# Parcels-code/Parcels

Hardware: AMD Instinct MI355X
Metric: RK4 particle-steps/sec (higher is better)
Workload: dtype f64

## Files before the change

parcels_amd/csrc/pk_api.hip:

```cpp
#include "pk_api_ctx.h"

#include <rocprim/rocprim.hpp>

using namespace pkapi;

namespace pkapi {
std::string g_init_error;
}

namespace pk {

PK_DEV unsigned long long order_double(double v) {
    unsigned long long b = (unsigned long long)__double_as_longlong(v);
    return (b & 0x8000000000000000ull) ? ~b : (b | 0x8000000000000000ull);
}

__global__ void __launch_bounds__(64) clock_probe_kernel(unsigned long long* out, unsigned long long ticks) {
    if (threadIdx.x != 0) return;
    const unsigned long long r0 = __builtin_amdgcn_s_memrealtime();
    const unsigned long long c0 = __builtin_readcyclecounter();
    unsigned long long r = r0;
    while (r - r0 < ticks) {
        __builtin_amdgcn_s_sleep(8);
        r = __builtin_amdgcn_s_memrealtime();
// ... 1701 lines not shown
    if (ok) {
        PK_HIP(ctx, hipStreamSynchronize(ctx->compute));
        if (tab.size() > t.cap) {
            if (t.d) PK_HIP(ctx, hipFree(t.d));
            PK_HIP(ctx, hipMalloc((void**)&t.d, tab.size() * sizeof(double)));
            t.cap = tab.size();
        }
        PK_HIP(ctx, hipMemcpy(t.d, tab.data(), tab.size() * sizeof(double), hipMemcpyHostToDevice));
    }
    t.ok = ok;
    return 0;
}

static int32_t fill_fast(pk_ctx* ctx, const pk_exec_params* prm, KArgs& a, int prog) {
    FastA& F = a.fast;
    memset(&F, 0, sizeof(F));
    if (ctx->no_fast || prm->interp_uv != 0 || prm->rk45_mode) return 0;
    const bool want_w = prog == PROG_RK4_3D;
    const HostField& U = ctx->fields[prm->fU];
    const HostField& V = ctx->fields[prm->fV];
    const HostField* W = (want_w && prm->fW >= 0) ? &ctx->fields[prm->fW] : nullptr;
    if (want_w && !W) return 0;
    const HostGrid& g = ctx->grids[U.d.grid];
    if (g.d.kind != 0 || g.d.lon_f32 || g.d.lat_f32 || g.d.depth_f32) return 0;
    if (V.d.grid != U.d.grid || (W && W->d.grid != U.d.grid)) return 0;
    auto same = [](const DField& x, const DField& y) { return x.ncomp == 1 && y.ncomp == 1 && same_layout(x, y); };
    if (!same(U.d, V.d) || (W && !same(U.d, W->d))) return 0;
    if (V.time != U.time || (W && W->time != U.time)) return 0;
    const DField& f = U.d;
    const size_t esz = f.dtype == PK_F64 ? 8 : 4;
    if (!g.d.has_x || f.st_x != 1 || f.nx < 2 || f.nx != g.d.nx) return 0;
    const bool fy = f.ny >= 2 && f.st_y > 0, fz = f.nz >= 2 && f.st_z > 0;
    if (fy && !(g.d.has_y && f.ny == g.d.ny)) return 0;
    if (fz && !(g.d.has_z && f.nz == g.d.nz)) return 0;
    if (f.has_time_interval && (f.nt < 2 || U.time.front() != 0.0)) return 0;
    const uint64_t lvl_b = (uint64_t)f.st_t * esz;
    const uint64_t last_b = ((uint64_t)f.nz * (uint64_t)f.st_z + (uint64_t)f.ny * (uint64_t)f.st_y + (uint64_t)f.nx) * esz;
    if (lvl_b >= (1ull << 32) || last_b >= (1ull << 32)) return 0;
    const CoordTable& T = ctx->tab_a;
    if (int32_t rc = coord_table(ctx, ctx->tab_a, U.d.grid, prm->fU, U.time.data(), f.has_time_interval ? f.nt : 0,
                                 {{g.d.depth, g.d.has_z ? g.d.nz : 0}, {g.d.lat, g.d.has_y ? g.d.ny : 0}, {g.d.lon, g.d.nx}}, 60 * 1024))
        return rc;
    if (!T.ok) return 0;
    const double inv_deg2m = 1.0 / g.d.deg2m;
    if (!(g.d.deg2m > 1e-100 && g.d.deg2m < 1e100) || !std::isfinite(inv_deg2m)) return 0;
    F.grid = U.d.grid;
    F.has_ti = f.has_time_interval;
    F.has_z = g.d.has_z; F.has_y = g.d.has_y; F.has_x = g.d.has_x;
    F.spherical = g.d.spherical;
    F.nt = f.nt;
    F.nslots = f.nslots;
    F.gnz = g.d.nz; F.gny = g.d.ny; F.gnx = g.d.nx;
    ravel_strides(g.d, F.ex, F.ey, F.ez);
    F.st_z = (uint32_t)f.st_z;
    F.st_y = (uint32_t)f.st_y;
    F.dyb = fy ? (uint32_t)(f.st_y * esz) : 0u;
    F.dzb = fz ? (uint32_t)(f.st_z * esz) : 0u;
    F.lds_time = T.off[0]; F.lds_depth = T.off[1]; F.lds_lat = T.off[2]; F.lds_lon = T.off[3];
    F.lds_n = T.off[4];
    F.lvl_b = (int64_t)lvl_b;
    F.U = (const char*)U.d.data; F.V = (const char*)V.d.data; F.W = W ? (const char*)W->d.data : nullptr;
    F.tab = T.d;
    F.tlen = f.tlen; F.t0 = f.tfirst; F.t1 = f.tlast;
    F.z0 = g.d.zfirst; F.z1 = g.d.zlast; F.y0 = g.d.yfirst; F.y1 = g.d.ylast; F.x0 = g.d.xfirst; F.x1 = g.d.xlast;
    F.deg2m = g.d.deg2m;
    F.inv_deg2m = inv_deg2m;
    F.ok = 1;
    return 0;
}

static void ensure_velocity_pairs(pk_ctx* ctx, const pk_exec_params* prm, FastC& F) {
    F.vp = nullptr;
    F.vp_slot_b = 0;
    F.vp_hi = 0;
    if (ctx->no_velocity_pairs) return;
    const HostField& U = ctx->fields[prm->fU];
    const HostField& V = ctx->fields[prm->fV];
    const DField& f = U.d;
    if (!f.has_time_interval || f.nt < 2 || f.st_t <= 0) return;
    const size_t esz = f.dtype == PK_F64 ? 8 : 4;
    const int ns = f.nslots;
    const size_t slot_b = (size_t)f.st_t * 8 * esz;
    const size_t need = slot_b * (size_t)ns;
    if (ctx->vp_fU != prm->fU || ctx->vp_fV != prm->fV || ctx->vp_bytes != need || (int)ctx->vp_level.size() != ns) {
        if (ctx->d_vp) {
            (void)hipStreamSynchronize(ctx->compute);
            (void)hipFree(ctx->d_vp);
            ctx->d_vp = nullptr;
        }
        ctx->vp_fU = prm->fU;
        ctx->vp_fV = prm->fV;
        ctx->vp_bytes = need;
        ctx->vp_level.assign(ns, -1);
        ctx->vp_gen.assign((size_t)ns * 4, 0);
        size_t free_b = 0, total_b = 0;
        if (hipMemGetInfo(&free_b, &total_b) != hipSuccess || free_b < need + std::max(need, total_b / 4)) {
            (void)hipGetLastError();
            ctx->d_vp = nullptr;
        } else if (hipMalloc((void**)&ctx->d_vp, need) != hipSuccess) {
            (void)hipGetLastError();
            ctx->d_vp = nullptr;
        }
    }
    if (!ctx->d_vp) return;
    const int64_t cb = F.cb;
    int lo = -1, hi = -1, count = 0;
// ... 664 lines not shown
```

parcels_amd/csrc/pk_device.h:

```cpp
#pragma once
#include <hip/hip_runtime.h>
#include <stdint.h>

#include "../../include/parcels_hip.h"

namespace pk {

struct DGrid {
    int32_t kind, spherical;
    int32_t has_x, has_y, has_z;
    int32_t nx, ny, nz;
    int32_t xdim, ydim, zdim;
    int32_t off_x, off_y, off_z;
    int32_t lon_f32, lat_f32, depth_f32;
    int32_t h_bitwidth;
    double deg2m;
    const double* lon;
    const double* lat;
    const double* depth;
    const double* node_tab;
    const double* cell_tab;
    const uint32_t* h_keys;
    const int64_t* h_starts;
    const int64_t* h_counts;
// ... 25 lines not shown
    int32_t ngrids, spatial_f32;
    double* t;
    void *z, *y, *x, *dz, *dy, *dx;
    double* dt;
    double* next_dt;
    int32_t* state;
    int32_t* ei;
    int64_t* particle_id;
    void* extra[PK_MAX_EXTRA];
    int32_t extra_f32[PK_MAX_EXTRA];
    int32_t* iter;
};

struct DPOut {
    double* t;
    void *z, *y, *x, *dz, *dy, *dx;
    double* dt;
    double* next_dt;
    int32_t* state;
    int32_t* ei;
    int32_t* iter;
};

struct DCounters {
    unsigned long long steps, attempts, paused;
    unsigned int err_iter, pad;
    unsigned long long twe_key;
    unsigned int twe_overflow, pad2;
    unsigned int pad3[20];
    unsigned int cursor[8 * 32];
};
constexpr int PK_CURSOR_STRIDE = 32;
static_assert(offsetof(DCounters, cursor) == 128, "the cursors start on a line of their own");

struct FastA {
    int32_t ok, grid;
    int32_t has_ti, has_z, has_y, has_x, spherical;
    int32_t nt, nslots;
    int32_t gnz, gny, gnx;
    uint32_t ex, ey, ez;
    uint32_t st_z, st_y;
    uint32_t dyb, dzb;
    int32_t lds_time, lds_depth, lds_lat, lds_lon, lds_n;
    int32_t lds_blk;
    int64_t lvl_b;
    const char *U, *V, *W;
    const double* tab;
    double tlen, t0, t1, z0, z1, y0, y1, x0, x1;
    double deg2m, inv_deg2m;
    int32_t ns;
    int32_t miss_lanes;
    int32_t sfid[4];
    const char* S[4];
};

struct FastC {
    int32_t ok, grid;
    int32_t has_ti, has_z, walk_ok, near_edges;
    int32_t nt, nslots;
    int32_t gnz, gny, gnx;
    uint32_t ex, ey, ez;
    int32_t lds_time, lds_depth, lds_n;
    int32_t lds_rec, lds_fv;
    int32_t st_z, st_y;
    int32_t cb;
    int64_t lvl_b;
    int64_t dU0, dU1, dV0, dV1;
    union { int64_t dW0; int64_t vp_slot_b; };
    union { int64_t dW1; int64_t vp_hi; };
    const char *U, *V;
    union { const char* W; const char* vp; };
    const char* kh[2];
    int32_t kh_st[2], kh_sz[2], kh_sy[2];
    int32_t kh_nt[2], kh_nz[2], kh_ny[2], kh_nx[2], kh_has_ti[2], kh_nslots[2];
    const double* ct2;
    const double* tab;
    double tlen, t0, t1, z0, z1, deg2m;
};

struct SigmaA {
    const double* tab;
    int32_t n;
    int32_t fh, fzeta;
    int32_t cs_f32;
    double hc;
};

#define PK_CONST_AS __attribute__((address_space(4)))
struct KArgs {
    const PK_CONST_AS DGrid* grids;
    const PK_CONST_AS DField* fields;
    DParticles p;
    pk_exec_params prm;
    double win_lo, win_hi;
    DCounters* counters;
    const unsigned long long* twe_listed;
    unsigned long long* twe_found;
    unsigned int* twe_hit;
    int32_t lds_time, lds_depth, lds_lat, lds_lon, lds_total;
    int32_t lds_cc_nodes, lds_cc_keys, lds_cc_fvals;
    int32_t main_grid, main_field;
    DPOut po;
    union {
        FastA fast;
        FastC fastc;
        SigmaA sigma;
    };
};

#define PK_DEV __device__ __forceinline__
PK_DEV const DGrid& kgrid(const KArgs& a, int g) { return *(const DGrid*)(a.grids + g); }
PK_DEV const DField& kfield(const KArgs& a, int f) { return *(const DField*)(a.fields + f); }
PK_DEV unsigned long long twe_sample_key(unsigned it, int klo) { return ((unsigned long long)it << 32) | (unsigned long long)(unsigned)klo; }
PK_DEV bool twe_listed(const KArgs& a, unsigned it, int klo) {
    const int n = a.prm.twe_n;
    if (__builtin_expect(n == 0, 1)) return false;
    const unsigned long long key = twe_sample_key(it, klo);
    const unsigned long long* lst = a.twe_listed;
    int lo = 0, hi = n;
    while (lo < hi) {
        const int mid = (lo + hi) >> 1;
        if (lst[mid] < key) lo = mid + 1; else hi = mid;
    }
    return it != 0 && lo < n && lst[lo] == key;
}
PK_DEV void twe_note(const KArgs& a, unsigned it, int klo) {
    if (it != 0) atomicMin(&a.counters->twe_key, twe_sample_key(it, klo));
}
constexpr int TWE_FOUND_SLOTS = 4096;
PK_DEV void twe_note_all(const KArgs& a, unsigned it, int klo) {
    if (it == 0) return;
    const unsigned long long key = twe_sample_key(it, klo);
    atomicMin(&a.counters->twe_key, key);
    unsigned h = (unsigned)((key * 0x9E3779B97F4A7C15ull) >> 52);
    for (int probe = 0; probe < TWE_FOUND_SLOTS; probe++) {
        unsigned long long* slot = a.twe_found + ((h + probe) & (TWE_FOUND_SLOTS - 1));
        unsigned long long cur = *(volatile unsigned long long*)slot;
        if (cur == key) return;
        if (cur == 0ull) {
            cur = atomicCAS(slot, 0ull, key);
            if (cur == 0ull || cur == key) return;
        }
    }
    atomicAdd(&a.counters->twe_overflow, 1u);
}
PK_DEV int twe_listed_index(const KArgs& a, unsigned it, int klo) {
    const int n = a.prm.twe_n;
    if (__builtin_expect(n == 0, 1)) return -1;
    const unsigned long long key = twe_sample_key(it, klo);
    const unsigned long long* lst = a.twe_listed;
    int lo = 0, hi = n;
    while (lo < hi) {
        const int mid = (lo + hi) >> 1;
        if (lst[mid] < key) lo = mid + 1; else hi = mid;
    }
    return (it != 0 && lo < n && lst[lo] == key) ? lo : -1;
}
PK_DEV void twe_justify(const KArgs& a, int idx, double t, double tlen) {
    if (!(0 <= t) || !(t <= tlen)) a.twe_hit[idx] = 1u;
}

// ... 1360 lines not shown
```

parcels_amd/csrc/pk_fast_agrid.h:

```cpp
#pragma once
#include "pk_device.h"

namespace pk {

typedef double pk_tab2 __attribute__((ext_vector_type(2)));

struct FastTabs {
    const pk_tab2* time;
    const pk_tab2* depth;
    const pk_tab2* lat;
    const pk_tab2* lon;
    pk_tab2* blk;
    uint32_t fl;
    double tlen;
    int32_t gny, gnx;
    double deg2m, inv_deg2m;
};
PK_DEV void copy_scalars(FastTabs& T, const FastA& F) {
    T.tlen = F.tlen;
    T.gny = F.gny;
    T.gnx = F.gnx;
}
enum : uint32_t {
    FA_TI = 1u, FA_Z = 2u, FA_Y = 4u, FA_X = 8u, FA_SPH = 16u, FA_RING = 32u, FA_BLK = 64u,
// ... 344 lines not shown
        const uint64_t addr = fbase + ((uint64_t)((mkey >> 2) + lbit) * (uint64_t)lvl_b + rowoff + (uint64_t)mb00);
        const uint32_t skip = (m >> 7) | (ln & 1u & ~mkey) | (lbit & ~(mkey >> 1));
        double cx = 0.0, cy = 0.0;
        if (skip == 0u) ldpair_at(addr, cx, cy, FT());
        const double dx = dpp_f64<DPP_XOR1, 0xf>(cx), dy = dpp_f64<DPP_XOR1, 0xf>(cy);
        const double zx = fma(mzeta, dx - cx, cx), zy = fma(mzeta, dy - cy, cy);
        const bool lenZ = (mkey & 1u) != 0;
        cx = lenZ ? zx : cx;
        cy = lenZ ? zy : cy;
        const double ax = dpp_f64<DPP_SHR4, 0xa>(cx), ay = dpp_f64<DPP_SHR4, 0xa>(cy);
        const bool lenT = (mkey & 2u) != 0;
        const double ex = lenT ? cx - ax : 0.0, ey = lenT ? cy - ay : 0.0;
        const bool l = lbit != 0;
        cx = l ? ex : cx;
        cy = l ? ey : cy;
        const double h = cy - cx;
        const double ox = dpp_f64<DPP_XOR2, 0xf>(cx), oh = dpp_f64<DPP_XOR2, 0xf>(h);
        const bool r = (ln & 2u) != 0;
        pk_tab2 e;
        e.x = r ? cx - ox : cx;
        e.y = r ? h - oh : h;
        if (((m >> 7) | (ln & 1u)) == 0u) (T.blk + ((int)m - (int)ln))[((ln >> 1) & 7u) * FAST_WG_LP] = e;
    } while (mm);
}

PK_DEV int fast_oob_state(int s, int xi, int yi, int zi, double xsi, double eta, double zeta, double tau) {
    if ((xi == RIGHT_OUT_OF_BOUNDS || yi == RIGHT_OUT_OF_BOUNDS || zi == RIGHT_OUT_OF_BOUNDS) && s < PK_ERROROUTOFBOUNDS) s = PK_ERROROUTOFBOUNDS;
    if (zi == LEFT_OUT_OF_BOUNDS && s < PK_ERRORTHROUGHSURFACE) s = PK_ERRORTHROUGHSURFACE;
    const bool bad = !(isfinite(xsi) && isfinite(eta) && isfinite(zeta) && isfinite(tau));
    if (bad && s < PK_ERRORINTERPOLATION) s = PK_ERRORINTERPOLATION;
    return s;
}

struct FCtx {
    int state;
    int32_t ei;
    int ht, hz, hy, hx;
    int zi;
    uint32_t zez;
    double mt, mtau, mz, mzeta;
    int32_t bei;
    int32_t bkey;
    double ya, yb, yr, xa, xb, xr;
    LpField fu, fv;
    double ta, tb, tr;
};
constexpr int32_t FAST_NO_BLOCK = -0x7fffffff - 1;
constexpr int FAST_Z_UNSEARCHED = -3;
constexpr int FAST_Z_UNSEARCHED_PACKED = -0x7fffffff - 1;
PK_DEV void fctx_depth_moved(FCtx& c, bool held) {
    c.zi = held ? FAST_Z_UNSEARCHED_PACKED : FAST_Z_UNSEARCHED;
    c.ya = __builtin_inf();
}
PK_DEV void fctx_init(FCtx& c, int state, int32_t ei, bool cache, bool held) {
    c.state = state;
    c.ei = ei;
    c.ht = c.hz = c.hy = c.hx = 0;
    c.zi = held ? FAST_Z_UNSEARCHED_PACKED : cache ? FAST_Z_UNSEARCHED : 0;
    c.ya = c.xa = c.ta = __builtin_inf();
    c.yb = c.xb = c.yr = c.xr = c.tb = c.tr = 0.0;
    c.zez = 0u;
    c.mt = c.mz = __builtin_nan("");
    c.mtau = c.mzeta = 0.0;
    c.bei = FAST_NO_BLOCK;
    c.bkey = -1;
    c.fu.p0 = c.fu.p1 = c.fu.d0 = c.fu.d1 = c.fv.p0 = c.fv.p1 = c.fv.d0 = c.fv.d1 = pk_tab2{0.0, 0.0};
}

PK_DEV bool fast_time_outside(const KArgs& a, const FastTabs& T, FCtx& c, double t, unsigned it, int klo) {
    const bool out = !(0 <= t) || !(t <= T.tlen);
    if (__builtin_expect(out, 0)) {
        c.state = PK_ERROROUTSIDETIMEINTERVAL;
        twe_note(a, it, klo);
    }
    return out;
}
PK_DEV void fast_time_memo(const FastTabs& T, const FastA& F, FCtx& c, uint32_t fl, double t, bool drop) {
    if (t != c.mt) {
        int idx;
        fast_search<true>(T.time, F.nt, F.t0, F.t1, t, c.ht, idx, c.mtau, (fl & FA_NT2) != 0);
        c.mt = t;
        if (drop) c.bei = FAST_NO_BLOCK;
    }
}
PK_DEV void fast_depth_search(const FastTabs& T, const FastA& F, FCtx& c, uint32_t fl, double z, bool keyed) {
    fast_search<true>(T.depth, F.gnz, F.z0, F.z1, z, c.hz, c.zi, c.mzeta, (fl & FA_NZ2) != 0);
    c.zez = (uint32_t)c.zi * F.ez;
    if (keyed) c.mz = z;
    c.bei = FAST_NO_BLOCK;
}
constexpr uint32_t FA_YX2 = FA_Y | FA_X | FA_NY2 | FA_NX2;
PK_DEV bool fast_search_yx(const FastTabs& T, const FastA& F, FCtx& c, uint32_t fl, double y, double x, int zi, double zeta, double tau, int& yi,
                           int& xi, double& eta, double& xsi) {
    if ((fl & FA_YX2) == FA_YX2) {
        fast_search2(T.lat, T.gny, F.y0, F.y1, y, c.hy, yi, eta, T.lon, T.gnx, F.x0, F.x1, x, c.hx, xi, xsi);
    } else {
        if (fl & FA_Y) fast_search<true>(T.lat, T.gny, F.y0, F.y1, y, c.hy, yi, eta, (fl & FA_NY2) != 0);
        if (fl & FA_X) fast_search<true>(T.lon, T.gnx, F.x0, F.x1, x, c.hx, xi, xsi, (fl & FA_NX2) != 0);
    }
    c.ei = (int32_t)((uint32_t)xi + __umul24((uint32_t)yi, F.ey) + c.zez);
    const bool out = (xi | yi | zi) < 0;
    if (__builtin_expect(out, 0)) {
        c.ei = (int32_t)((uint32_t)xi + (uint32_t)yi * F.ey + c.zez);
        c.state = fast_oob_state(c.state, xi, yi, zi, xsi, eta, zeta, tau);
    }
    return out;
}
template <bool PF, bool STEP>
PK_DEV void fast_convert(const FastTabs& T, const FastA& F, double y, bool pos_f32, double& uu, double& vv) {
    double conv;
    if (PF && pos_f32) conv = (double)((float)F.deg2m * cosf((float)y * DEG2RADF));
    else if constexpr (STEP) conv = T.deg2m * cos_lat_lean(y);
    else if constexpr (PK_FAST_LEAN != 0) conv = F.deg2m * cos_lat_lean(y);
    else conv = F.deg2m * cos_lat(y * DEG2RAD);
    if constexpr (PK_FAST_LEAN != 0) {
        uu = uu * rcp_lean(conv);
        vv = vv * (STEP ? T.inv_deg2m : F.inv_deg2m);
    } else {
        uu /= conv;
// ... 68 lines not shown
        }
        if (keep) c.bei = c.ei;
    }
    if (fl & FA_SPH) fast_convert<PF, false>(T, F, y, pos_f32, uu, vv);
    fast_nan_state(c, uu, vv, ww);
    u = uu;
    v = vv;
    w = ww;
}

template <class FT, bool PF, int LP>
PK_DEV void eval_uvw_lp(const KArgs& a, const FastTabs& T, FCtx& c, double t, double z, double y, double x, bool pos_f32, double& u, double& v,
                        unsigned it, int klo) {
    static_assert(LP == FAST_LP_REGS || LP == FAST_LP_CACHE, "a level-pair mode (2-D: z must not move inside a step)");
    const FastA& F = a.fast;
    uint32_t fl = T.fl;
    asm volatile("" : "+s"(fl));
    u = v = 0.0;
    constexpr bool CACHE = LP == FAST_LP_CACHE, HELD = fast_held(LP, PF);
    LpField fu, fv;
    int ti = 0;
    double tau = 0.0;
    if (fl & FA_TI) {
        if (fast_time_outside(a, T, c, t, it, klo)) return;
        if constexpr (HELD) {
            if (__builtin_expect((c.ta < t) & (t <= c.tb), 1)) {
                tau = fast_bary(t, c.ta, c.tb, c.tr);
            } else {
                int idx;
                pk_tab2 e;
                double a1;
                const bool two = (fl & FA_NT2) != 0;
                fast_search<true>(T.time, F.nt, F.t0, F.t1, t, c.ht, idx, tau, two, &e, &a1);
                c.ta = __builtin_inf();
                if (two && idx >= 0) { c.ta = e.x; c.tb = a1; c.tr = e.y; }
            }
        } else {
            fast_time_memo(T, F, c, fl, t, false);
            tau = c.mtau;
        }
        ti = c.ht;
    }
    int zi = 0, yi = 0, xi = 0;
    double zeta = 0.0, eta = 0.0, xsi = 0.0;
    auto depth_zeta = [&]() -> double {
        if ((fl & (FA_Z | FA_NZ2)) != (FA_Z | FA_NZ2)) return 0.0;
        const int q = c.zi >> 1;
        const int h = q >= 0 ? q : (q == LEFT_OUT_OF_BOUNDS ? 0 : F.gnz - 2);
        const pk_tab2 e = T.depth[h];
        return fast_bary(z, e.x, T.depth[h + 1].x, e.y);
    };
    if (fl & FA_Z) {
        if constexpr (HELD) {
            if (c.zi == FAST_Z_UNSEARCHED_PACKED) {
                int hz = 0, idx;
                double bz;
                fast_search<true>(T.depth, F.gnz, F.z0, F.z1, z, hz, idx, bz, (fl & FA_NZ2) != 0);
                c.zi = idx * 2 + (!(bz <= 0) ? 1 : 0);
                c.bei = FAST_NO_BLOCK;
            }
            zi = c.zi >> 1;
        } else {
            if (CACHE ? c.zi == FAST_Z_UNSEARCHED : !(z == c.mz)) {
                fast_depth_search(T, F, c, fl, z, !CACHE);
            }
            zi = c.zi;
            zeta = c.mzeta;
        }
    }
    if constexpr (CACHE) {
        const bool yx2 = (fl & FA_YX2) == FA_YX2;
        const bool same = yx2 & (c.ya < y) & (y <= c.yb) & (c.xa < x) & (x <= c.xb);
        if (__builtin_expect(same, 1)) {
            eta = fast_bary(y, c.ya, c.yb, c.yr);
            xsi = fast_bary(x, c.xa, c.xb, c.xr);
        } else {
            CellEntries e;
            if (yx2) {
                fast_search2(T.lat, T.gny, F.y0, F.y1, y, c.hy, yi, eta, T.lon, T.gnx, F.x0, F.x1, x, c.hx, xi, xsi, &e);
            } else {
                if (fl & FA_Y) fast_search<true>(T.lat, T.gny, F.y0, F.y1, y, c.hy, yi, eta, (fl & FA_NY2) != 0);
                if (fl & FA_X) fast_search<true>(T.lon, T.gnx, F.x0, F.x1, x, c.hx, xi, xsi, (fl & FA_NX2) != 0);
            }
            c.ei = (int32_t)((uint32_t)xi + (uint32_t)yi * F.ey + (HELD ? (uint32_t)zi * F.ez : c.zez));
            if (__builtin_expect((xi | yi | zi) < 0, 0)) {
                if (HELD) zeta = depth_zeta();
                c.state = fast_oob_state(c.state, xi, yi, zi, xsi, eta, zeta, tau);
                c.ya = __builtin_inf();
                return;
            }
            if (yx2) {
                c.ya = e.ea.x; c.yb = e.a1a; c.yr = e.ea.y;
                c.xa = e.eb.x; c.xb = e.a1b; c.xr = e.eb.y;
            }
        }
        yi = c.hy;
        xi = c.hx;
    } else {
        if (fast_search_yx(T, F, c, fl, y, x, zi, zeta, tau, yi, xi, eta, xsi)) return;
    }
    const bool lenT = tau > 0, lenZ = HELD ? (c.zi & 1) != 0 : !(zeta <= 0);
    const int key = (ti << 2) | (lenT ? 2 : 0) | (!HELD && lenZ ? 1 : 0);
    const uint32_t b00 = ((uint32_t)zi * F.st_z + (uint32_t)yi * F.st_y + (uint32_t)xi) * (uint32_t)sizeof(FT);
    double uu = 0.0, vv = 0.0;
    const bool miss = !CACHE || c.ei != c.bei || key != c.bkey;
    const bool some_miss = !CACHE || __builtin_amdgcn_ballot_w64(miss) != 0;
    if (some_miss) {
        if (HELD) zeta = depth_zeta();
// ... 129 lines not shown
```

parcels_amd/csrc/pk_kernels.h:

```cpp
#pragma once
#include "pk_device.h"
#include "pk_fast_agrid.h"
#include "pk_fast_cgrid.h"

namespace pk {

static_assert(sizeof(KArgs) <= 4096, "kernel arguments must fit the 4 KiB kernarg segment");

enum Program { PROG_RK4 = 0, PROG_RK4_3D = 1, PROG_GENERIC = 2, PROG_RK45 = 3, PROG_M1 = 4, PROG_TYPED = 5 };

struct PState {
    double t, z, y, x, dz, dy, dx, dt, next_dt;
    int64_t id;
};

PK_DEV double ldp(const void* col, int64_t i, bool pf) { return pf ? (double)((const float*)col)[i] : ((const double*)col)[i]; }
PK_DEV void stp(void* col, int64_t i, double v, bool pf) {
    if (pf) ((float*)col)[i] = (float)v; else ((double*)col)[i] = v;
}
PK_DEV double padd(bool pf, double a, double b) { return pf ? (double)((float)a + (float)b) : a + b; }
PK_DEV double psub(bool pf, double a, double b) { return pf ? (double)((float)a - (float)b) : a - b; }
PK_DEV double pstore(bool pf, double v) { return pf ? (double)(float)v : v; }

enum { RQ_UV = 0, RQ_UVW = 1, RQ_SCALAR = 2 };
// ... 303 lines not shown
                case 4: L.r[5] = u; break;
                case 5: L.r[6] = u; break;
                default: L.r[7] = u; break;
            }
            break;
        case PK_KERNEL_DIFFUSION_UNIFORM_KH:
            if (stage == 0) L.r[0] = u; else L.r[1] = u;
            break;
        case PK_KERNEL_SAMPLE_FIELD:
            L.r[0] = u; L.r[1] = v; L.r[2] = w;
            break;
        default:
            L.r[3] = u; L.r[4] = v; L.r[5] = w;
            break;
    }
}

PK_DEV void note_error_iteration(const KArgs& a, int state, unsigned it) {
    if (state >= PK_ERROR || state == PK_STOPALLEXECUTION) atomicMin(&a.counters->err_iter, it);
}

PK_DEV unsigned long long wave_sum(unsigned long long v) {
#pragma unroll
    for (int off = 32; off > 0; off >>= 1) v += __shfl_xor(v, off, 64);
    return v;
}

PK_DEV unsigned long long uniform_u64(unsigned long long v) {
    const unsigned lo = (unsigned)__builtin_amdgcn_readfirstlane((int)(unsigned)v), hi = (unsigned)__builtin_amdgcn_readfirstlane((int)(unsigned)(v >> 32));
    return ((unsigned long long)hi << 32) | lo;
}

PK_DEV unsigned xcd_swizzle(unsigned bid, unsigned nb) {
    const unsigned xcd = bid & 7u, j = bid >> 3;
    const unsigned per = nb >> 3, rem = nb & 7u;
    return xcd * per + (xcd < rem ? xcd : rem) + j;
}

constexpr int FAST_CHUNK = 64;
PK_DEV bool fast_claim(DCounters* cnt, unsigned nchunks, unsigned& tried, unsigned& chunk) {
    const unsigned per = nchunks >> 3, rem = nchunks & 7u;
    while (tried < 8u) {
        const unsigned s = (blockIdx.x + tried) & 7u;
        unsigned k = 0u;
        if ((threadIdx.x & 63) == 0) k = atomicAdd(&cnt->cursor[s * PK_CURSOR_STRIDE], 1u);
        k = (unsigned)__builtin_amdgcn_readfirstlane((int)k);
        if (k < per + (s < rem ? 1u : 0u)) {
            chunk = s * per + (s < rem ? s : rem) + k;
            return true;
        }
        tried++;
    }
    return false;
}

#ifndef PK_MIN_WAVES
#define PK_MIN_WAVES 1
#endif
#ifndef PK_MIN_WAVES_HEAVY
#define PK_MIN_WAVES_HEAVY 2
#endif
template <class FT, int KIND, int INTERP, int KID, bool LDS, bool TYPED, int PFM = -1>
__global__ void __launch_bounds__(wg_size(KIND, LDS), (KIND == 1 || INTERP != 0) ? PK_MIN_WAVES_HEAVY : PK_MIN_WAVES) advect_kernel(const KArgs a) {
    constexpr int WG = wg_size(KIND, LDS);
    extern __shared__ __attribute__((aligned(16))) double smem[];
    const DField& mf = kfield(a, a.main_field);
    const DGrid& mg = kgrid(a, a.main_grid);
    Coords mc;
    if (LDS) {
        double* s_time = smem + a.lds_time;
        double* s_depth = smem + a.lds_depth;
        double* s_lat = smem + a.lds_lat;
        double* s_lon = smem + a.lds_lon;
        const int nt = mf.has_time_interval ? mf.nt : 0;
        for (int k = threadIdx.x; k < nt; k += WG) s_time[k] = mf.time[k];
        const int nz = mg.has_z ? mg.nz : 0;
        for (int k = threadIdx.x; k < nz; k += WG) s_depth[k] = mg.depth[k];
        if (KIND == 0) {
            for (int k = threadIdx.x; k < mg.ny; k += WG) s_lat[k] = mg.lat[k];
            for (int k = threadIdx.x; k < mg.nx; k += WG) s_lon[k] = mg.lon[k];
        }
        __syncthreads();
        mc.time = s_time;
        mc.depth = s_depth;
        mc.lat = (KIND == 0) ? s_lat : mg.lat;
        mc.lon = (KIND == 0) ? s_lon : mg.lon;
    } else {
        mc.time = mf.time;
        mc.depth = mg.depth;
        mc.lat = mg.lat;
        mc.lon = mg.lon;
    }
    mc.cc.nodes = nullptr;
    mc.cc.key = nullptr;
    mc.cc.fvals = nullptr;
    if (LDS && KIND == 1 && a.lds_cc_nodes >= 0) {
        mc.cc.nodes = smem + a.lds_cc_nodes + threadIdx.x;
        mc.cc.key = (int*)(smem + a.lds_cc_keys) + threadIdx.x;
        if (INTERP == 1 && a.lds_cc_fvals >= 0) mc.cc.fvals = (void*)((FT*)(smem + a.lds_cc_fvals) + threadIdx.x);
        mc.cc.key[0] = -1;
        mc.cc.key[CC_LANES] = -1;
    }
    mc.t0 = mf.tfirst;
    mc.t1 = mf.tlast;
    mc.z0 = mg.zfirst; mc.z1 = mg.zlast;
    mc.y0 = mg.yfirst; mc.y1 = mg.ylast;
// ... 206 lines not shown
#pragma unroll 1
    for (int stage = 0; !user_prepare(a, kid - PK_KERNEL_USER0, stage, kslot, c, p, L, rq); stage++) {
        double u = 0.0, v = 0.0, w = 0.0;
        fc.state = c.state;
        if (rq.kind == RQ_SCALAR) {
            int slot = 0;
            for (int k = 1; k < a.fast.ns; k++) slot = a.fast.sfid[k] == rq.fidx ? k : slot;
            u = eval_scalar_fast<FT, PF>(a, ft, fc, slot, rq.t, rq.z, rq.y, rq.x, it, kslot * 1000 + stage);
        } else {
            eval_uvw_fast<FT, PF, D3>(a, ft, fc, rq.t, rq.z, rq.y, rq.x, PF && rq.f32, u, v, w, it, kslot * 1000 + stage);
        }
        c.state = fc.state;
        L.r[3] = u; L.r[4] = v; L.r[5] = w;
    }
    t = p.t; z = p.z; y = p.y; x = p.x; dz = p.dz; dy = p.dy; dx = p.dx; dt = p.dt;
    fc.state = c.state;
}
#endif

#ifndef PK_MIN_WAVES_FAST
#define PK_MIN_WAVES_FAST 4
#endif
template <class FT, int PFM, bool D3, int LP = FAST_LP_OFF>
__global__ void __launch_bounds__(fast_wg(LP), PK_MIN_WAVES_FAST) advect_fast_kernel(const KArgs a) {
    extern __shared__ __attribute__((aligned(16))) double smem[];
    constexpr int WG = fast_wg(LP);
    FastTabs ft;
    {
        pk_tab2* s_tab = reinterpret_cast<pk_tab2*>(smem);
        const pk_tab2* g_tab = reinterpret_cast<const pk_tab2*>(a.fast.tab);
        for (int k = threadIdx.x; k < a.fast.lds_n; k += WG) s_tab[k] = g_tab[k];
        __syncthreads();
        ft.time = s_tab + a.fast.lds_time;
        ft.depth = s_tab + a.fast.lds_depth;
        ft.lat = s_tab + a.fast.lds_lat;
        ft.lon = s_tab + a.fast.lds_lon;
        ft.blk = s_tab + a.fast.lds_blk + threadIdx.x;
        copy_scalars(ft, a.fast);
        ft.fl = fast_flags(a.fast) | ((a.win_lo > -INFINITY || a.win_hi < INFINITY) ? FA_WIN : 0u) | (a.prm.dt0 > 0 ? FA_FWD : 0u) |
                (a.prm.max_iters > 0 ? FA_MAXIT : 0u);
        if constexpr (fast_held(LP, PFM == 1)) ft.fl |= (uint32_t)a.fast.miss_lanes << FA_MISS_LANES_SHIFT;
    }
    constexpr bool PERS = LP == FAST_LP_CACHE;
    [[maybe_unused]] unsigned chunk = 0u, tried = 0u;
    [[maybe_unused]] const unsigned nchunks = PERS ? (unsigned)((a.p.n + FAST_CHUNK - 1) / FAST_CHUNK) : 0u;
    auto row = [&]() {
        if constexpr (PERS) {
            unsigned tid = threadIdx.x;
            asm volatile("" : "+v"(tid));
            return (int64_t)chunk * FAST_CHUNK + (tid & 63u);
        } else return (int64_t)xcd_swizzle(blockIdx.x, gridDim.x) * WG + threadIdx.x;
    };
    [[maybe_unused]] unsigned long long all_steps = 0ull, all_attempts = 0ull, all_paused = 0ull;
    do {
        if constexpr (PERS) {
            if (!fast_claim(a.counters, nchunks, tried, chunk)) break;
        }
        unsigned steps = 0, attempts = 0, paused = 0;
        if (row() < a.p.n) {
            int64_t i = row();
            const DParticles& P = a.p;
            const DPOut& O = a.po;
            const pk_exec_params& prm = a.prm;
            constexpr bool pf = PFM == 1;
            FCtx c;
            c.state = prm.reset_state ? PK_EVALUATE : P.state[i];
            if (c.state == PK_EVALUATE) {
                unsigned it = prm.reset_state ? 0u : (unsigned)P.iter[i];
                fctx_init(c, PK_EVALUATE, P.ei[i * P.ngrids + a.fast.grid], LP == FAST_LP_CACHE, fast_held(LP, pf));
                double pt = P.t[i];
                double pz = ldp(P.z, i, pf), py = ldp(P.y, i, pf), px = ldp(P.x, i, pf);
                double pdz = ldp(P.dz, i, pf), pdy = ldp(P.dy, i, pf), pdx = ldp(P.dx, i, pf);
                double pdt = P.dt[i];
                const double endtime = prm.endtime;
                while (c.state == PK_EVALUATE) {
                    uint32_t fl = ft.fl;
                    asm volatile("" : "+s"(fl));
                    if constexpr (fast_held(LP, pf)) {
                        ft.deg2m = a.fast.deg2m;
                        ft.inv_deg2m = a.fast.inv_deg2m;
                        asm volatile("" : "+s"(ft.deg2m), "+s"(ft.inv_deg2m));
                    }
                    const bool fwd = (fl & FA_FWD) != 0;
                    const double tte = fwd ? endtime - pt : -(endtime - pt);
                    if (!(tte >= 0)) break;
                    if ((fl & FA_MAXIT) && it >= (unsigned)prm.max_iters) break;
                    double dtc;
                    if (fwd) dtc = fmax(fmin(pdt, tte), 0.0);
                    else dtc = fmin(fmax(pdt, -tte), 0.0);
                    if (fl & FA_WIN) {
                        const double t1 = pt + dtc;
                        const double lo = fmin(pt, t1), hi = fmax(pt, t1);
                        if (lo < a.win_lo || hi > a.win_hi) { paused = 1; break; }
                    }
                    it++;
                    pdt = dtc;
                    attempts++;
#ifdef PK_USER_KERNELS
                    int adv = 0;
                    for (; adv < prm.nk && !is_rk4_id(prm.kernels[adv]); adv++) {
                        attempts++;
                        side_kernel_fast<FT, pf, D3>(a, ft, c, prm.kernels[adv], adv, row(), it, pt, pz, py, px, pdz, pdy, pdx, pdt);
                    }
#else
                    constexpr int adv = 0;
#endif
                    double su = 0.0, sv = 0.0, sw = 0.0, lu = 0.0, lv = 0.0, lw = 0.0;
                    constexpr bool peel = LP != FAST_LP_OFF;
                    if constexpr (peel) {
                        double u, v;
                        eval_uvw_lp<FT, pf, LP>(a, ft, c, pt, pz, py, px, pf, u, v, it, adv * 1000);
                        su = lu = u; sv = lv = v;
                    }
#pragma unroll 1
                    for (int stage = peel ? 1 : 0; stage < 4; stage++) {
                        double st = pt, sz = pz, sy = py, sx = px;
                        if (stage > 0) {
                            const double cdt = stage == 3 ? 1.0 : 0.5;
                            sx = px + lu * cdt * pdt;
                            sy = py + lv * cdt * pdt;
                            if (D3) sz = pz + lw * cdt * pdt;
                            st = pt + cdt * pdt;
                        }
                        double u, v, w = 0.0;
                        if constexpr (peel) eval_uvw_lp<FT, pf, LP>(a, ft, c, st, sz, sy, sx, pf && stage == 0, u, v, it, adv * 1000 + stage);
                        else eval_uvw_fast<FT, pf, D3>(a, ft, c, st, sz, sy, sx, pf && stage == 0, u, v, w, it, adv * 1000 + stage, (stage & 1) ? 2 : 1);
                        if constexpr (fast_held(LP, pf)) {
                            const double wgt = stage == 3 ? 1.0 : 2.0;
                            su = fma3s(wgt, u, su);
                            sv = fma3s(wgt, v, sv);
                        } else if (stage == 0) { su = u; sv = v; sw = w; }
                        else if (stage == 3) { su = su + u; sv = sv + v; sw = sw + w; }
                        else { su = su + 2 * u; sv = sv + 2 * v; sw = sw + 2 * w; }
                        lu = u; lv = v; lw = w;
                    }
                    constexpr double sixth = 1.0 / 6.0;
                    pdx = pstore(pf, pdx + (PK_FAST_LEAN ? su * sixth : div_by_recip(su, 6.0, sixth)) * pdt);
                    pdy = pstore(pf, pdy + (PK_FAST_LEAN ? sv * sixth : div_by_recip(sv, 6.0, sixth)) * pdt);
                    if (D3) pdz = pstore(pf, pdz + (PK_FAST_LEAN ? sw * sixth : div_by_recip(sw, 6.0, sixth)) * pdt);
                    for (int k = adv + 1; k < prm.nk; k++) {
                        const int kid = prm.kernels[k];
                        attempts++;
#ifdef PK_USER_KERNELS
                        if (kid >= PK_KERNEL_USER0) {
                            side_kernel_fast<FT, pf, D3>(a, ft, c, kid, k, row(), it, pt, pz, py, px, pdz, pdy, pdx, pdt);
                            continue;
                        }
#endif
                        if (kid == PK_KERNEL_DELETE_ON_ERROR) {
                            if (c.state >= PK_ERROR) c.state = PK_DELETE;
                        } else if (c.state == PK_ERROROUTOFBOUNDS || c.state == PK_ERRORTHROUGHSURFACE) {
                            c.state = PK_DELETE;
                        }
                    }
                    if (c.state == PK_EVALUATE || c.state == PK_SUCCESS) {
                        if (tte > 0 && pt + pdt == pt) {
                            c.state = PK_ERROR;
                            break;
                        }
                        px = padd(pf, px, pdx);
                        py = padd(pf, py, pdy);
                        if constexpr (LP == FAST_LP_CACHE) {
                            if (__builtin_expect(!(pdz == 0), 0)) fctx_depth_moved(c, fast_held(LP, pf));
                        }
                        pz = padd(pf, pz, pdz);
                        pt += pdt;
                        pdx = pdy = pdz = 0.0;
                        steps++;
                    }
                    pdt = prm.dt0;
                    if (c.state == PK_EVALUATE && pt == endtime) c.state = PK_ENDOFLOOP;
                }
                i = row();
                asm volatile("" : "+v"(i));
                O.t[i] = pt;
                stp(O.z, i, pz, pf);
                stp(O.y, i, py, pf);
                stp(O.x, i, px, pf);
                stp(O.dz, i, pdz, pf);
                stp(O.dy, i, pdy, pf);
                stp(O.dx, i, pdx, pf);
                O.dt[i] = pdt;
                if (P.next_dt && O.next_dt != P.next_dt) O.next_dt[i] = P.next_dt[i];
                O.state[i] = c.state;
                for (int g = 0; g < P.ngrids; g++) O.ei[i * P.ngrids + g] = g == a.fast.grid ? c.ei : P.ei[i * P.ngrids + g];
                O.iter[i] = (int32_t)it;
                note_error_iteration(a, c.state, it);
            }
        }
        unsigned long long wsteps = wave_sum((unsigned long long)steps), wattempts = wave_sum((unsigned long long)attempts),
                           wpaused = wave_sum((unsigned long long)paused);
        if constexpr (PERS) {
            all_steps += uniform_u64(wsteps);
            all_attempts += uniform_u64(wattempts);
            all_paused += uniform_u64(wpaused);
            continue;
        }
        if ((threadIdx.x & 63) == 0) {
            if (wsteps) atomicAdd(&a.counters->steps, wsteps);
            if (wattempts) atomicAdd(&a.counters->attempts, wattempts);
            if (wpaused) atomicAdd(&a.counters->paused, wpaused);
        }
    } while (PERS);
    if constexpr (PERS) {
        if ((threadIdx.x & 63) == 0) {
            if (all_steps) atomicAdd(&a.counters->steps, all_steps);
            if (all_attempts) atomicAdd(&a.counters->attempts, all_attempts);
            if (all_paused) atomicAdd(&a.counters->paused, all_paused);
        }
    }
}


#ifndef PK_MIN_WAVES_CGRID
#define PK_MIN_WAVES_CGRID 3
#endif
#ifndef PK_MIN_WAVES_CGRID_RK45
#define PK_MIN_WAVES_CGRID_RK45 3
#endif
#ifndef PK_MIN_WAVES_CGRID_M1
#define PK_MIN_WAVES_CGRID_M1 3
#endif
#ifndef PK_CG_CACHE
#define PK_CG_CACHE 2
#endif
#ifndef PK_CG_CACHE_RK45
#define PK_CG_CACHE_RK45 60
#endif
#ifndef PK_CG_CACHE_M1
#define PK_CG_CACHE_M1 4
#endif
constexpr int CG_CACHE_RK4 = PK_CG_CACHE, CG_CACHE_RK45 = PK_CG_CACHE_RK45, CG_CACHE_M1 = PK_CG_CACHE_M1;
template <class FT, int PFM, bool D3, bool NE>
__global__ void __launch_bounds__(FC_LANES, PK_MIN_WAVES_CGRID) advect_cgrid_kernel(const KArgs a) {
    extern __shared__ __attribute__((aligned(16))) double smem[];
    const FastC& F = a.fastc;
    CgLds L;
    {
        pk_tab2* s_tab = reinterpret_cast<pk_tab2*>(smem);
        const pk_tab2* g_tab = reinterpret_cast<const pk_tab2*>(F.tab);
        for (int k = threadIdx.x; k < F.lds_n; k += FC_LANES) s_tab[k] = g_tab[k];
// ... 560 lines not shown
```

Measured before the change: 52.35 billion.

## Prefetch next chunk's particles, warm search hints, and flatten wave sums

```diff
diff --git a/parcels_amd/csrc/pk_api.hip b/parcels_amd/csrc/pk_api.hip
--- a/parcels_amd/csrc/pk_api.hip
+++ b/parcels_amd/csrc/pk_api.hip
@@ -1777,6 +1777,9 @@
     F.nslots = f.nslots;
     F.gnz = g.d.nz; F.gny = g.d.ny; F.gnx = g.d.nx;
     ravel_strides(g.d, F.ex, F.ey, F.ez);
+    auto rcp32 = [](uint32_t d) { return d == 0u ? 0u : (uint32_t)std::min<uint64_t>(((1ull << 32) + d - 1) / d, 0xffffffffull); };
+    F.ey_rcp = rcp32(F.ey);
+    F.ez_rcp = rcp32(F.ez);
     F.st_z = (uint32_t)f.st_z;
     F.st_y = (uint32_t)f.st_y;
     F.dyb = fy ? (uint32_t)(f.st_y * esz) : 0u;
diff --git a/parcels_amd/csrc/pk_device.h b/parcels_amd/csrc/pk_device.h
--- a/parcels_amd/csrc/pk_device.h
+++ b/parcels_amd/csrc/pk_device.h
@@ -101,6 +101,7 @@
     int32_t miss_lanes;
     int32_t sfid[4];
     const char* S[4];
+    uint32_t ey_rcp, ez_rcp;
 };
 
 struct FastC {
@@ -156,6 +157,7 @@
         SigmaA sigma;
     };
 };
+static_assert(sizeof(FastA) <= sizeof(FastC), "FastA grew past FastC: the kernel arguments of every kernel change their layout");
 
 #define PK_DEV __device__ __forceinline__
 PK_DEV const DGrid& kgrid(const KArgs& a, int g) { return *(const DGrid*)(a.grids + g); }
diff --git a/parcels_amd/csrc/pk_fast_agrid.h b/parcels_amd/csrc/pk_fast_agrid.h
--- a/parcels_amd/csrc/pk_fast_agrid.h
+++ b/parcels_amd/csrc/pk_fast_agrid.h
@@ -420,6 +420,9 @@
     c.zi = held ? FAST_Z_UNSEARCHED_PACKED : FAST_Z_UNSEARCHED;
     c.ya = __builtin_inf();
 }
+#ifndef PK_FAST_NO_BLOCK_FILL
+#define PK_FAST_NO_BLOCK_FILL 1
+#endif
 PK_DEV void fctx_init(FCtx& c, int state, int32_t ei, bool cache, bool held) {
     c.state = state;
     c.ei = ei;
@@ -432,7 +435,31 @@
     c.mtau = c.mzeta = 0.0;
     c.bei = FAST_NO_BLOCK;
     c.bkey = -1;
-    c.fu.p0 = c.fu.p1 = c.fu.d0 = c.fu.d1 = c.fv.p0 = c.fv.p1 = c.fv.d0 = c.fv.d1 = pk_tab2{0.0, 0.0};
+    if (!(held && PK_FAST_NO_BLOCK_FILL != 0)) c.fu.p0 = c.fu.p1 = c.fu.d0 = c.fu.d1 = c.fv.p0 = c.fv.p1 = c.fv.d0 = c.fv.d1 = pk_tab2{0.0, 0.0};
+}
+
+#ifndef PK_FAST_WARM_HINTS
+#define PK_FAST_WARM_HINTS 1
+#endif
+constexpr int FAST_Z_HINT_END = FAST_Z_UNSEARCHED_PACKED + 0x10000;
+PK_DEV uint32_t hint_div(uint32_t e, uint32_t d, uint32_t rcp, uint32_t& rem) {
+    uint32_t q = __umulhi(e, rcp);
+    uint32_t r = e - q * d;
+    if ((int32_t)r < 0 && d != 0u) { q--; r += d; }
+    if (r >= d && d != 0u) { q++; r -= d; }
+    rem = r;
+    return q;
+}
+PK_DEV int hint_clamp(uint32_t q, int n) { return (int)min(q, (uint32_t)max(n - 2, 0)); }
+PK_DEV void fctx_warm_hints(FCtx& c, const PK_CONST_AS FastA* F, int32_t ei, bool held) {
+    uint32_t r1, r0;
+    const uint32_t zq = hint_div((uint32_t)ei, F->ez, F->ez_rcp, r1);
+    const uint32_t yq = hint_div(r1, F->ey, F->ey_rcp, r0);
+    c.hy = hint_clamp(yq, F->gny);
+    c.hx = hint_clamp(r0, F->gnx);
+    const int hz = hint_clamp(zq, F->gnz);
+    if (held) c.zi = FAST_Z_UNSEARCHED_PACKED + hz;
+    else c.hz = hz;
 }
 
 PK_DEV bool fast_time_outside(const KArgs& a, const FastTabs& T, FCtx& c, double t, unsigned it, int klo) {
@@ -607,8 +634,8 @@
     };
     if (fl & FA_Z) {
         if constexpr (HELD) {
-            if (c.zi == FAST_Z_UNSEARCHED_PACKED) {
-                int hz = 0, idx;
+            if (PK_FAST_WARM_HINTS ? c.zi < FAST_Z_HINT_END : c.zi == FAST_Z_UNSEARCHED_PACKED) {
+                int hz = PK_FAST_WARM_HINTS ? c.zi - FAST_Z_UNSEARCHED_PACKED : 0, idx;
                 double bz;
                 fast_search<true>(T.depth, F.gnz, F.z0, F.z1, z, hz, idx, bz, (fl & FA_NZ2) != 0);
                 c.zi = idx * 2 + (!(bz <= 0) ? 1 : 0);
diff --git a/parcels_amd/csrc/pk_kernels.h b/parcels_amd/csrc/pk_kernels.h
--- a/parcels_amd/csrc/pk_kernels.h
+++ b/parcels_amd/csrc/pk_kernels.h
@@ -379,6 +379,37 @@
         tried++;
     }
     return false;
+}
+#ifndef PK_FAST_CLAIM_AHEAD
+#define PK_FAST_CLAIM_AHEAD 1
+#endif
+constexpr unsigned FAST_NO_CHUNK = ~0u;
+PK_DEV const PK_CONST_AS KArgs* fast_kernargs() {
+    const PK_CONST_AS char* p = (const PK_CONST_AS char*)__builtin_amdgcn_kernarg_segment_ptr();
+    asm volatile("" : "+s"(p));
+    return (const PK_CONST_AS KArgs*)p;
+}
+PK_DEV unsigned fast_claim_ahead(DCounters* cnt, unsigned nchunks, unsigned& tried) {
+    if (tried >= 8u) return FAST_NO_CHUNK;
+    const unsigned per = nchunks >> 3, rem = nchunks & 7u;
+    const unsigned s = (blockIdx.x + tried) & 7u;
+    unsigned k = 0u;
+    if ((threadIdx.x & 63) == 0) k = atomicAdd(&cnt->cursor[s * PK_CURSOR_STRIDE], 1u);
+    k = (unsigned)__builtin_amdgcn_readfirstlane((int)k);
+    if (k < per + (s < rem ? 1u : 0u)) return s * per + (s < rem ? s : rem) + k;
+    tried++;
+    return FAST_NO_CHUNK;
+}
+
+#ifndef PK_FAST_FLAT_SUMS
+#define PK_FAST_FLAT_SUMS 1
+#endif
+PK_DEV unsigned long long wave_sum_flat(unsigned v) {
+    const uint64_t nz = __builtin_amdgcn_ballot_w64(v != 0u);
+    if (nz == 0ull) return 0ull;
+    const unsigned first = (unsigned)__builtin_amdgcn_readlane((int)v, __builtin_ctzll(nz));
+    if (__builtin_amdgcn_ballot_w64((v != first) & (v != 0u)) == 0ull) return (unsigned long long)first * (unsigned)__builtin_popcountll(nz);
+    return uniform_u64(wave_sum((unsigned long long)v));
 }
 
 #ifndef PK_MIN_WAVES
@@ -691,11 +722,38 @@
         } else return (int64_t)xcd_swizzle(blockIdx.x, gridDim.x) * WG + threadIdx.x;
     };
     [[maybe_unused]] unsigned long long all_steps = 0ull, all_attempts = 0ull, all_paused = 0ull;
+    [[maybe_unused]] int warm_ht = 0;
+    constexpr bool AHEAD = PERS && PK_FAST_CLAIM_AHEAD != 0;
+    [[maybe_unused]] unsigned next_chunk = FAST_NO_CHUNK;
+    if constexpr (AHEAD) {
+        if (!fast_claim(a.counters, nchunks, tried, next_chunk)) next_chunk = FAST_NO_CHUNK;
+    }
     do {
-        if constexpr (PERS) {
+        if constexpr (AHEAD) {
+            if (next_chunk == FAST_NO_CHUNK) break;
+            chunk = next_chunk;
+        } else if constexpr (PERS) {
             if (!fast_claim(a.counters, nchunks, tried, chunk)) break;
         }
         unsigned steps = 0, attempts = 0, paused = 0;
+        [[maybe_unused]] int pre_state;
+        [[maybe_unused]] int32_t pre_ei, pre_iter;
+        [[maybe_unused]] double pre_t, pre_z, pre_y, pre_x, pre_dz, pre_dy, pre_dx, pre_dt;
+        if constexpr (AHEAD) {
+            constexpr bool pf = PFM == 1;
+            const PK_CONST_AS KArgs* ka = fast_kernargs();
+            const PK_CONST_AS DParticles& P = ka->p;
+            const int64_t i = row() < P.n ? row() : P.n - 1;
+            const bool reset = ka->prm.reset_state != 0;
+            pre_state = reset ? PK_EVALUATE : P.state[i];
+            pre_iter = reset ? 0 : P.iter[i];
+            pre_ei = P.ei[i * P.ngrids + ka->fast.grid];
+            pre_t = P.t[i];
+            pre_z = ldp(P.z, i, pf); pre_y = ldp(P.y, i, pf); pre_x = ldp(P.x, i, pf);
+            pre_dz = ldp(P.dz, i, pf); pre_dy = ldp(P.dy, i, pf); pre_dx = ldp(P.dx, i, pf);
+            pre_dt = P.dt[i];
+            next_chunk = fast_claim_ahead(ka->counters, nchunks, tried);
+        }
         if (row() < a.p.n) {
             int64_t i = row();
             const DParticles& P = a.p;
@@ -703,14 +761,27 @@
             const pk_exec_params& prm = a.prm;
             constexpr bool pf = PFM == 1;
             FCtx c;
-            c.state = prm.reset_state ? PK_EVALUATE : P.state[i];
+            if constexpr (AHEAD) c.state = pre_state;
+            else c.state = prm.reset_state ? PK_EVALUATE : P.state[i];
             if (c.state == PK_EVALUATE) {
-                unsigned it = prm.reset_state ? 0u : (unsigned)P.iter[i];
-                fctx_init(c, PK_EVALUATE, P.ei[i * P.ngrids + a.fast.grid], LP == FAST_LP_CACHE, fast_held(LP, pf));
-                double pt = P.t[i];
-                double pz = ldp(P.z, i, pf), py = ldp(P.y, i, pf), px = ldp(P.x, i, pf);
-                double pdz = ldp(P.dz, i, pf), pdy = ldp(P.dy, i, pf), pdx = ldp(P.dx, i, pf);
-                double pdt = P.dt[i];
+                unsigned it;
+                int32_t ei0;
+                if constexpr (AHEAD) { it = (unsigned)pre_iter; ei0 = pre_ei; }
+                else { it = prm.reset_state ? 0u : (unsigned)P.iter[i]; ei0 = P.ei[i * P.ngrids + a.fast.grid]; }
+                fctx_init(c, PK_EVALUATE, ei0, LP == FAST_LP_CACHE, fast_held(LP, pf));
+                if constexpr (PERS && PK_FAST_WARM_HINTS != 0) {
+                    fctx_warm_hints(c, &fast_kernargs()->fast, ei0, fast_held(LP, pf));
+                    c.ht = warm_ht;
+                }
+                double pt, pz, py, px, pdz, pdy, pdx, pdt;
+                if constexpr (AHEAD) {
+                    pt = pre_t; pz = pre_z; py = pre_y; px = pre_x; pdz = pre_dz; pdy = pre_dy; pdx = pre_dx; pdt = pre_dt;
+                } else {
+                    pt = P.t[i];
+                    pz = ldp(P.z, i, pf); py = ldp(P.y, i, pf); px = ldp(P.x, i, pf);
+                    pdz = ldp(P.dz, i, pf); pdy = ldp(P.dy, i, pf); pdx = ldp(P.dx, i, pf);
+                    pdt = P.dt[i];
+                }
                 const double endtime = prm.endtime;
                 while (c.state == PK_EVALUATE) {
                     uint32_t fl = ft.fl;
@@ -810,6 +881,7 @@
                     pdt = prm.dt0;
                     if (c.state == PK_EVALUATE && pt == endtime) c.state = PK_ENDOFLOOP;
                 }
+                if constexpr (PERS && PK_FAST_WARM_HINTS != 0) warm_ht = c.ht;
                 i = row();
                 asm volatile("" : "+v"(i));
                 O.t[i] = pt;
@@ -826,6 +898,15 @@
                 O.iter[i] = (int32_t)it;
                 note_error_iteration(a, c.state, it);
             }
+        }
+        if constexpr (AHEAD) {
+            if (next_chunk == FAST_NO_CHUNK && !fast_claim(a.counters, nchunks, tried, next_chunk)) next_chunk = FAST_NO_CHUNK;
+        }
+        if constexpr (PERS && PK_FAST_FLAT_SUMS != 0) {
+            all_steps += wave_sum_flat(steps);
+            all_attempts += wave_sum_flat(attempts);
+            all_paused += wave_sum_flat(paused);
+            continue;
         }
         unsigned long long wsteps = wave_sum((unsigned long long)steps), wattempts = wave_sum((unsigned long long)attempts),
                            wpaused = wave_sum((unsigned long long)paused);
```

Measured after the change: 52.40 billion (median of 3 runs). About the same (+0.1%).
